# spcl/EBCC

Measured on AMD Instinct MI355X. Metric: fp32 GB/s encode+decode, 721x1440 ERA5 frames MAX_ERROR=0.5, higher is better.
Workload: dtype f32; 1 GPU; 256-frame batch 721x1440 fp32 per GPU, base_cr=30 MAX_ERROR=0.5 (BASELINE configs[1]); frames_per_gpu=256, parallelism=frames sharded over 1 GPU(s), no collective, hw_queues=4, encode_slices=3

## Files before the change

ebcc_amd/csrc/batch_codec.hip:

```cpp
#include "host.hpp"

namespace ebcc {
namespace {

DevRateSearch rate_search_start(float cr0, double q_init, double q_target)
{
    DevRateSearch r{};
    r.lo = r.hi = r.cr = cr0; r.q = r.q0 = q_init; r.qt = q_target;
    r.last.cr = -1; r.last.complete = 1;
    return r;
}

struct Job {
    bool const_field = false;
    float minv = 0, maxv = 0, target = -1, cr = -1;
    double mean_err = 0, q = 0, q_first = 0;
    float rmin = 0, rmax = 0;
    bool skip = true, need_pure = false;
    float best_err = -1;
    size_t coeffs_orig = 0, coeffs_size = 0, len1 = 0;
    double t_hi = 0, t_lo = 0, t_best = 0;
    bool trunc_active = false;
    std::vector<uint8_t> tail, zbytes;
    DevRateSearch rs[2] = {};
    std::vector<DevProbe> probes;
};

struct Batch {
    ebcc_hip_ctx *ctx;
    J2kBuffers &jb;
    const float *d_frames;
    size_t n, tiles, nt;
    std::vector<J2kFrame> jf;
    J2kFrame *tjf;
    std::vector<int> active;
    int *tactive, *ractive;
    std::vector<float> state_cr;
    int *d_active;
    hipStream_t s;
    ebcc_hip_ctx *rc;
    hipStream_t rs;
    Batch(ebcc_hip_ctx *c, const float *d, size_t n_, size_t tiles_ = 1, ebcc_hip_ctx *rc_ = nullptr)
        : ctx(c), jb(*static_cast<J2kBuffers *>(c->j2k)), d_frames(d), n(n_), tiles(tiles_), nt(n_ * tiles_), jf(n_),
          tjf(static_cast<J2kFrame *>(c->h_jf)), active(n_, 0), tactive(c->h_act), ractive(c->h_act + c->max_frames), state_cr(n_, -1.f),
          d_active(c->d_active), s(c->stream), rc(rc_ ? rc_ : c), rs((rc_ ? rc_ : c)->stream)
    {
// ... 26 lines not shown
    {
        for (size_t c = 0; c < n; c++)
            for (size_t t = c * tiles; t < (c + 1) * tiles; t++) tactive[t] = active[c];
        EBCC_HIP_CHECK(hipMemcpyAsync(d_active, tactive, sizeof(int) * nt, hipMemcpyHostToDevice, s));
    }
    void push_ractive()
    {
        for (size_t c = 0; c < n; c++) ractive[c] = active[c];
        EBCC_HIP_CHECK(hipMemcpyAsync(rc->d_active, ractive, sizeof(int) * n, hipMemcpyHostToDevice, rs));
    }
    void allocate()
    {
        push_jf();
        push_active();
        launch_j2k_rate(jb, (int) nt, d_active, s);
    }
    void probe(bool decode)
    {
        allocate();
        if (decode) launch_j2k_probe_decode(d_frames, jb, (int) nt, d_active, s);
        fetch_jf();
    }
    template <class Jobs>
    void collect_tails(Jobs &jobs)
    {
        push_active();
        launch_j2k_write(jb, (int) nt, d_active, s);
        fetch_jf();
        if (tiles == 1) {
            std::vector<size_t> len(n, 0), off(n, 0);
            for (size_t f = 0; f < n; f++) if (active[f]) len[f] = (size_t) jf[f].stream_bytes;
            stage_download(ctx, jb.stream, jb.stream_cap, len.data(), off.data(), n, s);
            for (size_t f = 0; f < n; f++)
                if (active[f]) jobs[f].tail.assign(ctx->h_stage + off[f], ctx->h_stage + off[f] + len[f]);
            return;
        }
        for (size_t c = 0; c < n; c++) {
            if (!active[c]) continue;
            std::vector<uint8_t> &o = jobs[c].tail;
            o.resize((size_t) jf[c].stream_bytes);
            size_t at = kJ2kMainHeaderBytes;
            for (size_t k = 0; k < tiles; k++) {
                const size_t t = c * tiles + k, part = 14 + (size_t) tjf[t].body_bytes;
                const uint8_t *slot = jb.stream + t * jb.stream_cap;
                if (k == 0) EBCC_HIP_CHECK(hipMemcpyAsync(o.data(), slot, kJ2kMainHeaderBytes, hipMemcpyDeviceToHost, s));
                EBCC_HIP_CHECK(hipMemcpyAsync(o.data() + at, slot + kJ2kMainHeaderBytes, part, hipMemcpyDeviceToHost, s));
                at += part;
            }
        }
        wait_stream(s);
        const unsigned H = (unsigned) jb.geom.H;
        for (size_t c = 0; c < n; c++) {
            if (!active[c]) continue;
            std::vector<uint8_t> &o = jobs[c].tail;
            auto put32 = [&](size_t at, unsigned v) { o[at] = (uint8_t) (v >> 24); o[at + 1] = (uint8_t) (v >> 16); o[at + 2] = (uint8_t) (v >> 8); o[at + 3] = (uint8_t) v; };
            put32(12, H * (unsigned) tiles);
            size_t at = kJ2kMainHeaderBytes;
            for (size_t k = 0; k < tiles; k++) {
                o[at + 4] = (uint8_t) (k >> 8); o[at + 5] = (uint8_t) k;
                at += 14 + (size_t) tjf[c * tiles + k].body_bytes;
            }
            o[at] = 0xFF; o[at + 1] = 0xD9;
        }
    }
};

int search_rounds() { const char *e = getenv("EBCC_HIP_SEARCH_ROUNDS"); return e ? std::max(1, atoi(e)) : 16; }
constexpr int kSearchAll = 0, kSearchStart = 1, kSearchFinish = 2;

struct Entropy {
    enum : uint8_t { kNone = 0, kQueued = 1, kRunning = 2, kSkipped = 3 };
    using PoolBatches = std::vector<std::shared_ptr<HostPool::Batch>>;
    std::vector<Job> &jobs;
    const unsigned slices;
    const int level;
    const bool timing, trace;
    std::vector<const uint8_t *> coeff_ptr;
    std::unique_ptr<std::atomic<uint8_t>[]> zstate;
    std::vector<size_t> zfloor;
    std::atomic<long long> zstd_us{0}, zstd_max_us{0}, zstd_bytes{0}, bound_us{0};
    long long wait_us = 0;
    PoolBatches zbatches, fbatches;

    Entropy(std::vector<Job> &j, unsigned slices_, int level_, bool timing_)
        : jobs(j), slices(slices_), level(level_), timing(timing_), trace(timing_ && getenv("EBCC_HIP_ZSTD_TRACE")),
          coeff_ptr(j.size(), nullptr), zstate(new std::atomic<uint8_t>[j.size()]), zfloor(j.size(), 0)
    { for (size_t f = 0; f < j.size(); f++) zstate[f] = kNone; }
    Entropy(const Entropy &) = delete; Entropy &operator=(const Entropy &) = delete;
    ~Entropy() { for (PoolBatches *v : {&fbatches, &zbatches}) for (auto &b : *v) if (b) b->wait(); }

    void submit_zstd(std::vector<size_t> list)
    {
        if (trace) fprintf(stderr, "zstd-submit batch %p jobs %zu\n", (const void *) &jobs, list.size());
        for (size_t f : list) zstate[f] = kQueued;
        auto order = std::make_shared<std::vector<size_t>>(std::move(list));
        zbatches.push_back(HostPool::instance().submit(order->size(), entropy_threads(slices), [this, order](size_t i) {
            const size_t f = (*order)[i];
            uint8_t expect = kQueued;
            if (!zstate[f].compare_exchange_strong(expect, kRunning)) return;
            Job &j = jobs[f];
            const auto z0 = std::chrono::steady_clock::now();
            j.zbytes.resize(zstd().bound(j.coeffs_size));
            const size_t z = zstd().compress(j.zbytes.data(), j.zbytes.size(), coeff_ptr[f], j.coeffs_size, level);
            if ((zstd().is_error && zstd().is_error(z)) || z > j.zbytes.size()) throw std::runtime_error("ZSTD_compress failed on a residual prefix");
            j.zbytes.resize(z);
            const long long us = std::chrono::duration_cast<std::chrono::microseconds>(std::chrono::steady_clock::now() - z0).count();
            if (trace) {
                static const auto epoch = std::chrono::steady_clock::now();
                const long long a = std::chrono::duration_cast<std::chrono::microseconds>(z0 - epoch).count();
                fprintf(stderr, "zstd-job batch %p bytes %zu start %lld us end %lld us cpu %d\n", (const void *) &jobs, j.coeffs_size, a, a + us, sched_getcpu());
            }
            zstd_us += us; zstd_bytes += (long long) j.coeffs_size;
            long long m = zstd_max_us.load(); while (us > m && !zstd_max_us.compare_exchange_weak(m, us)) {}
        }));
    }
    void submit_floors(const std::vector<size_t> &frames)
    {
        auto list = std::make_shared<std::vector<size_t>>(frames);
        fbatches.push_back(HostPool::instance().submit(list->size(), entropy_threads(slices), [this, list](size_t i) {
            const size_t f = (*list)[i];
            const auto z0 = std::chrono::steady_clock::now();
            zfloor[f] = zstd_size_lower_bound(coeff_ptr[f], jobs[f].coeffs_size);
            bound_us += std::chrono::duration_cast<std::chrono::microseconds>(std::chrono::steady_clock::now() - z0).count();
        }));
    }
    std::vector<size_t> longest_first(std::vector<size_t> list) const
    {
        std::stable_sort(list.begin(), list.end(), [&](size_t a, size_t c) { return jobs[a].coeffs_size > jobs[c].coeffs_size; });
        return list;
    }
    std::vector<size_t> lowest_floor_first(std::vector<size_t> list) const
    {
        std::stable_sort(list.begin(), list.end(), [&](size_t a, size_t c) {
            return (double) zfloor[a] * (double) jobs[c].coeffs_size < (double) zfloor[c] * (double) jobs[a].coeffs_size; });
        return list;
    }
// ... 5 lines not shown
    bool floor_decides(size_t f) const { return zfloor[f] > 0 && (size_t) jobs[f].rs[1].last.stream_bytes < zfloor[f] + jobs[f].len1; }
    bool strike(size_t f)
    {
        uint8_t expect = kNone;
        if (zstate[f].compare_exchange_strong(expect, kSkipped)) return true;
        expect = kQueued;
        return zstate[f].compare_exchange_strong(expect, kSkipped);
    }
    bool join(PoolBatches &v)
    {
        const auto w0 = std::chrono::steady_clock::now();
        bool ok = true;
        std::string why;
        for (auto &b : v) if (b && !b->wait()) { ok = false; if (why.empty()) why = b->error; }
        v.clear();
        wait_us += std::chrono::duration_cast<std::chrono::microseconds>(std::chrono::steady_clock::now() - w0).count();
        if (!ok) { log_fatal("entropy stage failed: %s", why.c_str()); set_error("%s", why.c_str()); }
        return ok;
    }
    bool join_floors() { return join(fbatches); }
    bool join_all() { const bool a = join(fbatches), c = join(zbatches); return a && c; }
    void report(const std::vector<size_t> &with_prefix, long long skipped, long long skipped_bytes) const
    {
        if (timing) fprintf(stderr, "ebcc-mi355x zstd: %.1f ms of core time for %lld bytes, longest job %.1f ms; floors %.1f ms; %lld of %zu prefixes (%lld bytes) not compressed\n",
                            zstd_us.load() / 1e3, zstd_bytes.load(), zstd_max_us.load() / 1e3, bound_us.load() / 1e3, skipped, with_prefix.size(), skipped_bytes);
        host_stats().skipped_bytes += skipped_bytes;
        if (trace)
            for (size_t f : with_prefix) {
                const Job &j = jobs[f];
                const long long x = (long long) j.rs[1].last.stream_bytes - (long long) j.len1;
                fprintf(stderr, "zstd-trace c %zu floor %zu X %lld z %zu state %d need_pure %d nbad1 %llu len1 %zu orig %zu\n", j.coeffs_size, zfloor[f], x, j.zbytes.size(), (int) zstate[f].load(), (int) j.need_pure,
                        (unsigned long long) j.rs[0].last.nbad, j.len1, j.coeffs_orig);
            }
    }
};

struct BatchEncode {
    struct Gate { SliceGate *g; void release() { if (g) { g->release(); g = nullptr; } } ~Gate() { release(); } } next;
    struct NoteOnce { PhaseNote *n; void tell() { if (n) { n->slice_done(); n = nullptr; } } ~NoteOnce() { tell(); } } gpu_phase_over;
    const EncodeEnv env;
    const codec_config_t *cfg;
    const int mode;
    const bool searching;
    const double q_target;
    const bool want_pure;
    const size_t n, n_pix;
    const unsigned slices;
    Batch b;
    const bool overlap2;
    std::vector<Job> jobs;
    PhaseTimer pt;
    bool any_resid = false;
    bool search2_queued = false;

    BatchEncode(ebcc_hip_ctx *ctx, const float *d_frames, size_t n_, const codec_config_t *cfg_, SliceGate *next_, size_t tiles,
                ebcc_hip_ctx *rctx, unsigned slices_, PhaseNote *note)
        : next{next_}, gpu_phase_over{note}, cfg(cfg_), mode((int) cfg_->residual_compression_type),
          searching(mode == MAX_ERROR || mode == RELATIVE_ERROR), q_target(1 - env.base_error_quantile),
          want_pure(q_target != 1.0 && !env.no_fallback), n(n_), n_pix(ctx->n_pix * tiles), slices(slices_),
          b(ctx, d_frames, n_, tiles, rctx), overlap2(want_pure && tiles == 1 && b.rc == ctx), jobs(n_) {}
    ~BatchEncode() { if (search2_queued && b.ctx->stream2) hipStreamSynchronize(b.ctx->stream2); }

    int analyse(); void first_probe(); void search_1(); void queue_search_2(); bool residual_layer(); void truncation_search();
    bool entropy_and_fallback(); int assemble(uint8_t **outs, size_t *sizes);
    void start_search_2();
    void rate_search(int k, int lane = 0, int part = kSearchAll);
};

void BatchEncode::rate_search(int k, int lane, int part)
{
    ebcc_hip_ctx *ctx = b.ctx;
    DevChunk *h = static_cast<DevChunk *>(ctx->h_search) + (size_t) lane * ctx->max_frames, *d = static_cast<DevChunk *>(ctx->d_search) + (size_t) lane * ctx->max_frames;
    int *const d_counter = ctx->d_counter + 4 * lane, *const h_counter = ctx->h_counter + 4 * lane;
    int *const d_active = lane ? ctx->d_active + ctx->max_frames : b.d_active;
    hipStream_t s = lane ? second_stream(ctx) : b.s;
    J2kBuffers &jb = b.jb;
    const int forced = getenv("EBCC_HIP_SPECULATION") ? atoi(getenv("EBCC_HIP_SPECULATION")) != 0 : -1;
    const bool speculate = lane == 0 && (forced >= 0 ? forced != 0 : slices <= 1);
    hipStream_t s2 = nullptr;
    double jobs_qt0 = 0.0;
    for (size_t f = 0; f < n; f++) if (!jobs[f].const_field) { jobs_qt0 = jobs[f].rs[0].qt; break; }
    const double limit_qt = getenv("EBCC_HIP_NO_SHORTCUTS") || g_log_level <= 0 ? 0.0 : std::min(jobs_qt0, 1.0);
    auto advance = [&]() {
        launch_search_advance(d, jb.jf, d_active, (int) n, (int) b.tiles, k, (double) n_pix, d_counter, s,
                              speculate ? jb.cand_cr : nullptr, speculate ? jb.cand_sel : nullptr, limit_qt);
        if (speculate) launch_j2k_rate_publish(jb, (int) b.nt, s);
    };
// ... 274 lines not shown
            drive(forced_rounds ? search_rounds() : cuts_left + 1, 6, [&] {
                launch_prefix_synthesis_stats(b.d_frames, b.jb.DEC, rc->rb, (int) n, rc->d_u64b, rc->d_active, rs);
                advance();
            });
        }
        for (size_t f = 0; f < n; f++) {
            Job &j = jobs[f];
            const DevChunk &c = h[f];
            if (j.trunc_active) { j.t_hi = c.t_hi; j.t_lo = c.t_lo; j.t_best = c.t_best; j.mean_err = c.mean_err; j.best_err = c.best_err; }
            j.trunc_active = false;
        }
    }
    for (Job &j : jobs) {
        if (j.const_field || j.skip) j.coeffs_size = j.need_pure ? j.coeffs_orig : 0;
        else j.coeffs_size = (size_t) (j.t_best / 8.);
    }
    pt.mark("truncation search");
}

bool BatchEncode::entropy_and_fallback()
{
    ebcc_hip_ctx *rc = b.rc;
    Entropy es(jobs, slices, env.zstd_level, pt.on);
    std::vector<size_t> coeff_len(n, 0), coeff_off(n, 0);
    for (size_t f = 0; f < n; f++) {
        if (jobs[f].coeffs_size <= 16) jobs[f].coeffs_size = 0;
        coeff_len[f] = jobs[f].coeffs_size;
    }
    stage_download(rc, (const uint8_t *) rc->rb.stream, rc->rb.stream_words * sizeof(uint32_t), coeff_len.data(), coeff_off.data(), n, b.rs);
    std::vector<size_t> with_prefix;
    for (size_t f = 0; f < n; f++)
        if (coeff_len[f]) { es.coeff_ptr[f] = rc->h_stage + coeff_off[f]; with_prefix.push_back(f); }
    std::vector<size_t> cand;
    if (!want_pure) {
        es.submit_zstd(es.longest_first(with_prefix));
    } else {
        const bool use_floor = zstd_floor_usable() && !getenv("EBCC_HIP_NO_SHORTCUTS");
        std::vector<size_t> now;
        for (size_t f : with_prefix) {
            if (jobs[f].need_pure) { es.zstate[f] = Entropy::kSkipped; continue; }
            (use_floor && jobs[f].coeffs_size <= kZstdFloorMaxBytes ? cand : now).push_back(f);
        }
        if (!now.empty()) es.submit_zstd(es.longest_first(now));
        if (!cand.empty()) es.submit_floors(cand);
    }
    pt.mark("zstd: queued");
    if (want_pure) {
        if (overlap2) {
            rate_search(1, 1, kSearchFinish);
            search2_queued = false;
            pt.mark("rate search 2");
            gpu_phase_over.tell();
            if (!es.join_floors()) return false;
        } else {
            start_search_2();
            rate_search(1, 0, kSearchStart);
            if (!cand.empty()) {
                if (!es.join_floors()) return false;
                es.submit_zstd(es.lowest_floor_first(cand));
            }
            rate_search(1, 0, kSearchFinish);
            pt.mark("rate search 2");
            gpu_phase_over.tell();
        }
        long long skipped_bytes = 0, skipped = 0;
        for (size_t f : cand)
            if (es.floor_decides(f) && es.strike(f)) { skipped++; skipped_bytes += (long long) jobs[f].coeffs_size; }
        if (overlap2) {
            const std::vector<size_t> open = es.not_started(cand);
            if (!open.empty()) es.submit_zstd(es.longest_first(open));
        }
        if (!es.join_all()) return false;
        pt.mark("zstd: wait for the workers");
        for (size_t f : with_prefix) if (jobs[f].need_pure) { skipped++; skipped_bytes += (long long) jobs[f].coeffs_size; }
        es.report(with_prefix, skipped, skipped_bytes);
        bool any_pure = false;
        for (size_t f = 0; f < n; f++) {
            Job &j = jobs[f];
            b.active[f] = 0;
            if (j.const_field) continue;
            const size_t len2 = (size_t) j.rs[1].last.stream_bytes;
            const bool decided = es.floor_decides(f);
            if (decided || len2 < j.zbytes.size() + j.len1 || j.need_pure) {
                if (decided) log_info("frame %zu: pure base compression (%zu) beats base (%zu) + residual (at least %zu)", f, len2, j.len1, es.zfloor[f]);
                else if (len2 < j.zbytes.size() + j.len1)
                    log_info("frame %zu: pure base compression (%zu) beats base (%zu) + residual (%zu)", f, len2, j.len1, j.zbytes.size());
                j.mean_err = j.rs[1].last.err_sum / (double) n_pix;
                j.zbytes.clear(); j.coeffs_size = 0;
                b.active[f] = 1; b.jf[f].cr = j.rs[1].result; any_pure = true;
            }
        }
        if (any_pure) { b.allocate(); b.collect_tails(jobs); }
    }
    if (!es.join_all()) return false;
    host_stats().add(es.zstd_us.load() + es.bound_us.load(), es.wait_us, es.zstd_bytes.load());
    return true;
}

int BatchEncode::assemble(uint8_t **outs, size_t *sizes)
{
    for (size_t f = 0; f < n; f++) {
        Job &j = jobs[f];
        float minv = j.minv, maxv = j.maxv;
        log_info("frame %zu: mean of compression error %e", f, j.mean_err);
        if (!env.no_mean_adjust && std::fabs(j.mean_err) > 1e-18) {
            minv += j.mean_err;
            maxv += j.mean_err;
        }
        const size_t codec_size = j.const_field ? sizeof(uint64_t) : j.tail.size();
        const size_t total = sizeof(FrameHeader) + j.zbytes.size() + codec_size;
        uint8_t *o = (uint8_t *) malloc(total), *p = o;
        if (!o) { log_fatal("out of memory"); return 1; }
        FrameHeader hd;
        memset(&hd, 0, sizeof hd);
        memcpy(hd.magic, EBCC_HEADER_MAGIC, 4);
        hd.version = EBCC_HEADER_VERSION;
        if (j.const_field) hd.flags |= EBCC_HEADER_FLAG_CONST_FIELD;
        hd.minval_bits = f2u(minv); hd.maxval_bits = f2u(maxv);
        hd.coeffs_size = j.coeffs_size;
        hd.rmin_bits = f2u(j.const_field ? 0.0f : j.rmin); hd.rmax_bits = f2u(j.const_field ? 0.0f : j.rmax);
        hd.compressed_size = j.zbytes.size(); hd.tail_size = codec_size;
        memcpy(p, &hd, sizeof hd); p += sizeof hd;
        if (!j.zbytes.empty()) { memcpy(p, j.zbytes.data(), j.zbytes.size()); p += j.zbytes.size(); }
        if (j.const_field) { uint64_t cnt = n_pix; memcpy(p, &cnt, 8); }
        else memcpy(p, j.tail.data(), j.tail.size());
        log_info("frame %zu: coeffs_size %zu compressed_size %zu jp2_length %zu ratio %f", f, j.coeffs_size, j.zbytes.size(),
                 codec_size, (double) (n_pix * 4) / (double) total);
        outs[f] = o;
        sizes[f] = total;
    }
    pt.mark("assemble");
    return 0;
}

}

int encode_batch(ebcc_hip_ctx *ctx, const float *d_frames, size_t n, const codec_config_t *cfg, uint8_t **outs, size_t *sizes,
                 SliceGate *next, size_t tiles, ebcc_hip_ctx *rctx, unsigned slices, PhaseNote *note)
{
    BatchEncode e(ctx, d_frames, n, cfg, next, tiles, rctx, slices, note);
    if (const int r = e.analyse()) return r;
    e.first_probe();
    if (e.searching) {
        e.search_1();
        e.queue_search_2();
        if (!e.residual_layer()) return 1;
        e.truncation_search();
        if (!e.entropy_and_fallback()) return 1;
    }
    e.pt.mark("fallback search + tails");
    return e.assemble(outs, sizes);
}
// ... 240 lines not shown
```

ebcc_amd/csrc/engine.hip:

```cpp
#include "engine.hpp"

#include <algorithm>
#include <atomic>
#include <cstdarg>
#include <mutex>
#include <string>
#include <type_traits>
#include <cstring>
#include <vector>

#include "../../include/ebcc_hip.h"
#include "search.hpp"

namespace ebcc {

static thread_local std::string g_last_error;

void set_error(const char *fmt, ...)
{
    char buf[512];
    va_list ap;
    va_start(ap, fmt);
    vsnprintf(buf, sizeof buf, fmt, ap);
    va_end(ap);
// ... 58 lines not shown
template float *ctx_alloc<float>(ebcc_hip_ctx *, size_t);
template int32_t *ctx_alloc<int32_t>(ebcc_hip_ctx *, size_t);
template uint32_t *ctx_alloc<uint32_t>(ebcc_hip_ctx *, size_t);
template uint16_t *ctx_alloc<uint16_t>(ebcc_hip_ctx *, size_t);
template uint8_t *ctx_alloc<uint8_t>(ebcc_hip_ctx *, size_t);
template double *ctx_alloc<double>(ebcc_hip_ctx *, size_t);
template unsigned long long *ctx_alloc<unsigned long long>(ebcc_hip_ctx *, size_t);
template FrameState *ctx_alloc<FrameState>(ebcc_hip_ctx *, size_t);

namespace {

__global__ __launch_bounds__(256) void k_stage(uint8_t *slots, size_t stride, const unsigned long long *pack, uint8_t *staged, int to_stage)
{
    const int f = blockIdx.x;
    const unsigned long long off = pack[2 * f], len = pack[2 * f + 1];
    if (!len) return;
    uint32_t *a = (uint32_t *) (slots + (size_t) f * stride), *b = (uint32_t *) (staged + off);
    const size_t words = (size_t) ((len + 3) / 4);
    for (size_t i = (size_t) blockIdx.y * blockDim.x + threadIdx.x; i < words; i += (size_t) gridDim.y * blockDim.x) {
        if (to_stage) b[i] = a[i]; else a[i] = b[i];
    }
}

size_t stage_layout(ebcc_hip_ctx *ctx, const size_t *len, size_t *off, size_t n)
{
    size_t total = 0;
    for (size_t f = 0; f < n; f++) {
        off[f] = total;
        ctx->h_pack[2 * f] = total; ctx->h_pack[2 * f + 1] = len[f];
        total += (len[f] + 15) & ~(size_t) 15;
    }
    if (total > ctx->stage_cap) {
        uint8_t *h_old = ctx->h_stage, *d_old = ctx->d_stage;
        ctx->h_stage = nullptr; ctx->d_stage = nullptr; ctx->stage_cap = 0;
        if (h_old) hipHostFree(h_old);
        if (d_old) hipFree(d_old);
        const size_t cap = total + total / 2 + 4096;
        uint8_t *h_new = nullptr, *d_new = nullptr;
        EBCC_HIP_CHECK(hipHostMalloc((void **) &h_new, cap));
        const hipError_t e = device_malloc((void **) &d_new, cap);
        if (e != hipSuccess) { hipHostFree(h_new); EBCC_HIP_CHECK(e); }
        ctx->h_stage = h_new; ctx->d_stage = d_new; ctx->stage_cap = cap;
        poison_alloc(d_new, cap);
    }
    return total;
}

}

void stage_download(ebcc_hip_ctx *ctx, const uint8_t *src, size_t stride, const size_t *len, size_t *off, size_t n, hipStream_t s)
{
    const size_t total = stage_layout(ctx, len, off, n);
    if (!total) return;
    EBCC_HIP_CHECK(hipMemcpyAsync(ctx->d_pack, ctx->h_pack, 2 * n * sizeof(unsigned long long), hipMemcpyHostToDevice, s));
    hipLaunchKernelGGL(k_stage, dim3((unsigned) n, 4), dim3(256), 0, s, const_cast<uint8_t *>(src), stride, ctx->d_pack, ctx->d_stage, 1);
    EBCC_HIP_CHECK(hipMemcpyAsync(ctx->h_stage, ctx->d_stage, total, hipMemcpyDeviceToHost, s));
    wait_stream(s);
}

void stage_reserve(ebcc_hip_ctx *ctx, const size_t *len, size_t *off, size_t m) { stage_layout(ctx, len, off, m); }

void stage_send(ebcc_hip_ctx *ctx, size_t m, hipStream_t s)
{
    size_t total = 0;
    for (size_t k = 0; k < m; k++) total = std::max<size_t>(total, ctx->h_pack[2 * k] + ((ctx->h_pack[2 * k + 1] + 15) & ~15ull));
    EBCC_HIP_CHECK(hipMemcpyAsync(ctx->d_pack, ctx->h_pack, 2 * m * sizeof(unsigned long long), hipMemcpyHostToDevice, s));
    if (total) EBCC_HIP_CHECK(hipMemcpyAsync(ctx->d_stage, ctx->h_stage, total, hipMemcpyHostToDevice, s));
}

void stage_scatter(ebcc_hip_ctx *ctx, uint8_t *dst, size_t stride, size_t first, size_t count, hipStream_t s)
{
    if (!count) return;
    hipLaunchKernelGGL(k_stage, dim3((unsigned) count, 4), dim3(256), 0, s, dst, stride, ctx->d_pack + 2 * first, ctx->d_stage, 0);
}

bool ensure_cut_slots(ebcc_hip_ctx *ctx, int capacity)
{
    if (ctx->cut.capacity >= capacity) return true;
    if (ctx->cut_failed) return false;
    const int cap = capacity;
// ... 201 lines not shown
{
    EBCC_API_TRY
    if (!ctx) return;
    hipSetDevice(ctx->device);
    if (ctx->stream) hipStreamSynchronize(ctx->stream);
    for (ebcc_hip_ctx *c : ctx->lanes) ebcc_hip_destroy(c);
    ctx->lanes.clear();
    if (ctx->twin) { ebcc_hip_destroy(ctx->twin); ctx->twin = nullptr; }
    j2k_destroy(ctx);
    for (void *p : ctx->allocs) hipFree(p);
    if (ctx->h_u64a) hipHostFree(ctx->h_u64a);
    if (ctx->h_u64b) hipHostFree(ctx->h_u64b);
    if (ctx->h_u64c) hipHostFree(ctx->h_u64c);
    if (ctx->h_active) hipHostFree(ctx->h_active);
    if (ctx->h_fs) hipHostFree(ctx->h_fs);
    if (ctx->h_pack) hipHostFree(ctx->h_pack);
    if (ctx->h_act) hipHostFree(ctx->h_act);
    if (ctx->h_search) hipHostFree(ctx->h_search);
    if (ctx->h_counter) hipHostFree(ctx->h_counter);
    if (ctx->h_jf) hipHostFree(ctx->h_jf);
    if (ctx->h_table) hipHostFree(ctx->h_table);
    if (ctx->h_stage) hipHostFree(ctx->h_stage);
    if (ctx->d_stage) hipFree(ctx->d_stage);
    if (ctx->d_io) hipFree(ctx->d_io);
    if (ctx->h_boxes) hipHostFree(ctx->h_boxes);
    if (ctx->d_boxes) hipFree(ctx->d_boxes);
    if (ctx->h_bounce) hipHostFree(ctx->h_bounce);
    if (ctx->ev_a) hipEventDestroy(ctx->ev_a);
    if (ctx->ev_b) hipEventDestroy(ctx->ev_b);
    if (ctx->stream2) hipStreamDestroy(ctx->stream2);
    if (ctx->stream) hipStreamDestroy(ctx->stream);
    delete ctx;
    EBCC_API_CATCH_VOID
}

void *ebcc_hip_stream(ebcc_hip_ctx *ctx) { return ctx ? (void *) ctx->stream : nullptr; }
size_t ebcc_hip_workspace_bytes(const ebcc_hip_ctx *ctx) { return ctx ? ctx->bytes : 0; }
size_t ebcc_hip_padded_pixels(const ebcc_hip_ctx *ctx) { return ctx ? ctx->rb.np : 0; }

void *ebcc_hip_malloc(size_t bytes)
{
    void *p = nullptr;
    if (device_malloc(&p, bytes ? bytes : 1) != hipSuccess) {
        set_error("ebcc_hip_malloc(%zu) failed", bytes);
        return nullptr;
    }
// ... 149 lines not shown
```

ebcc_amd/csrc/engine.hpp:

```cpp
#pragma once

#include <cstdint>
#include <string>
#include <vector>

#include "residual.hpp"

struct ebcc_hip_ctx {
    int device = 0;
    hipStream_t stream = nullptr;
    size_t max_frames = 0;
    int height = 0, width = 0;
    int tile_period = 1;
    size_t n_pix = 0;
    size_t bytes = 0;
    ebcc::ResidualBuffers rb{};
    unsigned long long *d_u64a = nullptr, *d_u64b = nullptr, *d_u64c = nullptr;
    int *d_active = nullptr;
    unsigned long long *h_u64a = nullptr, *h_u64b = nullptr, *h_u64c = nullptr;
    int *h_active = nullptr;
    ebcc::FrameState *h_fs = nullptr;
    void *h_jf = nullptr;
    int *h_act = nullptr;
    int *h_table = nullptr;
    void *d_search = nullptr, *h_search = nullptr;
    int *d_counter = nullptr, *h_counter = nullptr;
    std::vector<void *> allocs;
    void *j2k = nullptr;
    hipStream_t stream2 = nullptr;
    hipEvent_t ev_a = nullptr, ev_b = nullptr;
    std::vector<ebcc_hip_ctx *> lanes;
    ebcc_hip_ctx *twin = nullptr;
    bool twin_failed = false;
    uint8_t *h_stage = nullptr, *d_stage = nullptr;
    size_t stage_cap = 0;
    float *d_io = nullptr;
    size_t io_cap = 0;
    uint8_t *h_bounce = nullptr;
    unsigned long long *h_pack = nullptr, *d_pack = nullptr;
    void *h_boxes = nullptr, *d_boxes = nullptr;
    size_t boxes_cap = 0;
    ebcc::CutSlots cut{};
    bool cut_failed = false;
};

namespace ebcc {

void set_error(const char *fmt, ...);
ebcc_hip_ctx *create_engine(int device, size_t max_frames, size_t height, size_t width, int tile_period);
template <typename T>
T *ctx_alloc(ebcc_hip_ctx *ctx, size_t count);

void stage_download(ebcc_hip_ctx *ctx, const uint8_t *src, size_t stride, const size_t *len, size_t *off, size_t n, hipStream_t s);
void stage_reserve(ebcc_hip_ctx *ctx, const size_t *len, size_t *off, size_t m);
void stage_send(ebcc_hip_ctx *ctx, size_t m, hipStream_t s);
void stage_scatter(ebcc_hip_ctx *ctx, uint8_t *dst, size_t stride, size_t first, size_t count, hipStream_t s);

bool ensure_cut_slots(ebcc_hip_ctx *ctx, int capacity);

int check_ims_header(ebcc_hip_ctx *ctx, const uint8_t *b, size_t n, size_t num_bits);

void fetch_frame_states(ebcc_hip_ctx *ctx, size_t n_frames);
void push_frame_states(ebcc_hip_ctx *ctx, size_t n_frames, hipStream_t s = nullptr);

}
```

ebcc_amd/csrc/host.hpp:

```cpp
#pragma once

#include <dlfcn.h>

#include <chrono>
#include <cmath>
#include <cstdarg>
#include <cstring>
#include <ctime>
#include <sched.h>
#include <condition_variable>
#include <deque>
#include <functional>
#include <map>
#include <sys/mman.h>
#include <sys/resource.h>
#include <sys/syscall.h>
#include <unistd.h>
#include <tuple>
#include <algorithm>
#include <atomic>
#include <mutex>
#include <memory>
#include <thread>
#include <string>
#include <vector>

#include "../../include/ebcc_hip.h"
#include "engine.hpp"
#include "j2k.hpp"
#include "search.hpp"


namespace ebcc {

bool j2k_parse_codestream(const uint8_t *cs, size_t n, const J2kGeom &g, int *table);
bool j2k_peek_dims(const uint8_t *cs, size_t n, int *W, int *H, int *tile_w, int *tile_h);
bool j2k_parse_tiled(const uint8_t *cs, size_t n, const J2kBuffers &jb, int tiles, int *tables, size_t *part_off, size_t *part_len);

extern int g_log_level;
void log_at(int level, const char *fmt, ...);
#define log_trace(...) ::ebcc::log_at(0, __VA_ARGS__)
#define log_info(...) ::ebcc::log_at(2, __VA_ARGS__)
#define log_warn(...) ::ebcc::log_at(3, __VA_ARGS__)
#define log_fatal(...) ::ebcc::log_at(5, __VA_ARGS__)

struct Zstd {
    size_t (*bound)(size_t) = nullptr;
    size_t (*compress)(void *, size_t, const void *, size_t, int) = nullptr;
    size_t (*decompress)(void *, size_t, const void *, size_t) = nullptr;
    unsigned (*is_error)(size_t) = nullptr;
    unsigned (*version)(void) = nullptr;
    bool ok = false;
    Zstd();
};
Zstd &zstd();
constexpr size_t kZstdFloorMaxBytes = (size_t) 4 << 20;
bool zstd_floor_usable();
size_t zstd_size_lower_bound(const uint8_t *src, size_t n);

#pragma pack(push, 1)
struct FrameHeader {
    uint8_t magic[4]; uint8_t version; uint8_t flags; uint16_t reserved;
    uint32_t minval_bits, maxval_bits; uint64_t coeffs_size;
    uint32_t rmin_bits, rmax_bits; uint64_t compressed_size; uint64_t tail_size;
};
struct ChunkHeader {
    uint8_t magic[4]; uint32_t version, ndims, reserved;
    uint64_t dims[3], chunk_dims[3], num_chunks, chunk_size;
};
#pragma pack(pop)
static_assert(sizeof(FrameHeader) == 48, "EBCC header must be 48 bytes");
static_assert(sizeof(ChunkHeader) == 80, "EBCK header must be 80 bytes");
inline uint32_t f2u(float f) { uint32_t u; memcpy(&u, &f, 4); return u; }
inline float u2f(uint32_t u) { float f; memcpy(&f, &u, 4); return f; }

inline bool dims_are_valid(const size_t d[3])
{
    if (d[0] == 0 || d[1] == 0) return false;
    size_t hh = d[0] * d[1];
    if (hh / d[0] != d[1]) return false;
    return hh >= EBCC_MIN_INTERNAL_IMAGE_DIM && hh <= EBCC_MAX_INTERNAL_IMAGE_DIM && d[2] >= EBCC_MIN_INTERNAL_IMAGE_DIM &&
           d[2] <= EBCC_MAX_INTERNAL_IMAGE_DIM;
}

struct EncodeEnv {
    double base_error_quantile = 1e-6;
    bool no_fallback = false, no_consistency = false, no_mean_adjust = false;
    int zstd_level = 22;
    EncodeEnv()
    {
        if (const char *e = getenv("EBCC_INIT_BASE_ERROR_QUANTILE")) base_error_quantile = strtod(e, nullptr);
        no_fallback = getenv("EBCC_DISABLE_PURE_BASE_COMPRESSION_FALLBACK") != nullptr;
        no_consistency = getenv("EBCC_DISABLE_PURE_BASE_COMPRESSION_FALLBACK_CONSISTENCY") != nullptr;
        no_mean_adjust = getenv("EBCC_DISABLE_MEAN_ADJUSTMENT") != nullptr;
        if (const char *e = getenv("EBCC_ZSTD_LEVEL")) { long v = strtol(e, nullptr, 10); if (v >= 1 && v <= 22) zstd_level = (int) v; }
    }
};
// ... 13 lines not shown
struct SliceGate {
    std::mutex m;
    std::condition_variable cv;
    bool open = false;
    void release() { { std::lock_guard<std::mutex> l(m); open = true; } cv.notify_all(); }
    void wait() { std::unique_lock<std::mutex> l(m); cv.wait(l, [&] { return open; }); }
};

constexpr int kJ2kMainHeaderBytes = 135;

inline hipStream_t second_stream(ebcc_hip_ctx *c)
{
    if (!c->stream2) EBCC_HIP_CHECK(hipStreamCreateWithFlags(&c->stream2, hipStreamNonBlocking));
    return c->stream2;
}

double cgroup_cpu_quota();
unsigned usable_cpus();
unsigned entropy_threads_for(unsigned cpus, unsigned local_world, unsigned slices);
unsigned entropy_threads(unsigned slices = 1);

struct HostStats {
    std::atomic<long long> zstd_core_us{0}, zstd_wait_us{0}, zstd_bytes{0}, batches{0}, skipped_bytes{0};
    void add(long long core_us, long long wait_us, long long bytes) { zstd_core_us += core_us; zstd_wait_us += wait_us; zstd_bytes += bytes; batches++; }
    void reset() { zstd_core_us = 0; zstd_wait_us = 0; zstd_bytes = 0; batches = 0; skipped_bytes = 0; }
};
HostStats &host_stats();

class HostPool {
  public:
    struct Batch {
        std::function<void(size_t)> fn;
        size_t n = 0;
        std::atomic<size_t> next{0};
        std::atomic<size_t> left{0};
        std::atomic<bool> failed{false};
        std::string error;
        std::mutex m;
        std::condition_variable cv;
        void fail(const char *what) { std::lock_guard<std::mutex> l(m); if (!failed.exchange(true)) error = what; }
        bool wait()
        {
            work();
            std::unique_lock<std::mutex> l(m);
            cv.wait(l, [&] { return left.load() == 0; });
            return !failed.load();
        }
        void work()
// ... 105 lines not shown
```

ebcc_amd/csrc/host_codec.hip:

```cpp
#include "host.hpp"

using namespace ebcc;

namespace {

int resolve_device()
{
    int n = 0;
    if (hipGetDeviceCount(&n) != hipSuccess || n < 1) return 0;
    if (const char *e = getenv("EBCC_HIP_DEVICE")) { int d = atoi(e); return d >= 0 && d < n ? d : 0; }
    int d = 0;
    if (hipGetDevice(&d) != hipSuccess) d = 0;
    return d;
}
bool multi_process_job()
{
    for (const char *v : {"LOCAL_WORLD_SIZE", "WORLD_SIZE"})
        if (const char *e = getenv(v)) if (atoi(e) > 1) return true;
    return false;
}
std::vector<int> device_list()
{
    int n = 0;
    if (hipGetDeviceCount(&n) != hipSuccess || n < 1) return {0};
// ... 593 lines not shown
{
    static const char *names[] = {"NONE", "MAX_ERROR", "RELATIVE_ERROR"};
    log_info("dimensions:\t(%lu, %lu, %lu)", c->dims[0], c->dims[1], c->dims[2]);
    log_info("chunk dimensions:\t(%lu, %lu, %lu)", c->chunk_dims[0], c->chunk_dims[1], c->chunk_dims[2]);
    log_info("base_cr:\t%f", c->base_cr);
    unsigned t = (unsigned) c->residual_compression_type;
    log_info("residual type:\t%s", t < 3 ? names[t] : "?");
    if (t == MAX_ERROR) log_info("max error:\t%f", c->error);
    if (t == RELATIVE_ERROR) log_info("relative error:\t%f", c->error);
}

int ebcc_hip_host_threads(int slices) { return (int) entropy_threads((unsigned) std::max(1, slices)); }
int ebcc_hip_default_encode_slices(void) { return (int) default_encode_slices(); }
int ebcc_hip_encode_slices_for(size_t n_frames) { return (int) slice_count(n_frames, "EBCC_HIP_SLICES", default_encode_slices()); }

int ebcc_hip_selfcheck(void) { return j2k_selfcheck_div65535() + residual_selfcheck_divisions(); }
void ebcc_hip_plan_decode_lanes(const int *table, int n_code_blocks, int out[4]) { plan_decode_lanes(table, std::max(0, n_code_blocks), out); }

size_t ebcc_hip_zstd_floor(const uint8_t *src, size_t n) { return zstd_floor_usable() ? zstd_size_lower_bound(src, n) : 0; }

void ebcc_hip_host_stats(double *out, int reset)
{
    HostStats &h = host_stats();
    if (out) {
        out[0] = (double) usable_cpus(); out[1] = cgroup_cpu_quota();
        out[2] = h.zstd_core_us.load() / 1e6; out[3] = h.zstd_wait_us.load() / 1e6;
        out[4] = (double) h.zstd_bytes.load(); out[5] = (double) h.batches.load(); out[6] = (double) h.skipped_bytes.load();
    }
    if (reset) h.reset();
}

int ebcc_hip_upload(ebcc_hip_ctx *ctx, void *d_dst, const void *h_src, size_t bytes)
{
    if (!ctx || !d_dst || !h_src) { set_error("ebcc_hip_upload: null argument"); return 1; }
    return on_device(ctx->device, 1, [&] {
        copy_pageable(ctx, const_cast<void *>(h_src), d_dst, bytes, false);
        return 0;
    });
}
int ebcc_hip_download(ebcc_hip_ctx *ctx, void *h_dst, const void *d_src, size_t bytes)
{
    if (!ctx || !h_dst || !d_src) { set_error("ebcc_hip_download: null argument"); return 1; }
    return on_device(ctx->device, 1, [&] {
        huge_pages(h_dst, bytes);
        copy_pageable(ctx, h_dst, const_cast<void *>(d_src), bytes, true);
        return 0;
// ... 376 lines not shown
```

Baseline: 8.807 GB/s.

## Download pure codestreams early and assemble frames while zstd workers run

While zstd workers are still compressing residuals, the encoder now downloads the pure-base codestreams into a second staging buffer. It then assembles each frame as soon as both its payload and pure stream are ready, using a per-frame latch, so the choice and header assembly overlap with entropy coding instead of running after the join. This avoids a later GPU pass for fallback frames and moves assembly off the critical path. The cost is a speculative download of pure streams that may go unused, an extra pinned staging buffer, and assembly running from worker threads.

```diff
diff --git a/ebcc_amd/csrc/batch_codec.hip b/ebcc_amd/csrc/batch_codec.hip
--- a/ebcc_amd/csrc/batch_codec.hip
+++ b/ebcc_amd/csrc/batch_codec.hip
@@ -22,6 +22,12 @@
     double t_hi = 0, t_lo = 0, t_best = 0;
     bool trunc_active = false;
     std::vector<uint8_t> tail, zbytes;
+    const uint8_t *tail_pure = nullptr;
+    size_t tail_pure_len = 0;
+    FrameLatch latch;
+    uint8_t *out = nullptr;
+    size_t out_size = 0;
+    bool out_pure = false;
     DevRateSearch rs[2] = {};
     std::vector<DevProbe> probes;
 };
@@ -94,7 +100,7 @@
         fetch_jf();
     }
     template <class Jobs>
-    void collect_tails(Jobs &jobs)
+    size_t collect_tails(Jobs &jobs, bool beside = false)
     {
         push_active();
         launch_j2k_write(jb, (int) nt, d_active, s);
@@ -102,10 +108,16 @@
         if (tiles == 1) {
             std::vector<size_t> len(n, 0), off(n, 0);
             for (size_t f = 0; f < n; f++) if (active[f]) len[f] = (size_t) jf[f].stream_bytes;
+            if (beside) {
+                const size_t total = stage_download(ctx, jb.stream, jb.stream_cap, len.data(), off.data(), n, s, true);
+                for (size_t f = 0; f < n; f++)
+                    if (active[f]) { jobs[f].tail_pure = ctx->h_stage2 + off[f]; jobs[f].tail_pure_len = len[f]; }
+                return total;
+            }
             stage_download(ctx, jb.stream, jb.stream_cap, len.data(), off.data(), n, s);
             for (size_t f = 0; f < n; f++)
                 if (active[f]) jobs[f].tail.assign(ctx->h_stage + off[f], ctx->h_stage + off[f] + len[f]);
-            return;
+            return 0;
         }
         for (size_t c = 0; c < n; c++) {
             if (!active[c]) continue;
@@ -134,6 +146,7 @@
             }
             o[at] = 0xFF; o[at + 1] = 0xD9;
         }
+        return 0;
     }
 };
 
@@ -150,8 +163,9 @@
     std::vector<const uint8_t *> coeff_ptr;
     std::unique_ptr<std::atomic<uint8_t>[]> zstate;
     std::vector<size_t> zfloor;
-    std::atomic<long long> zstd_us{0}, zstd_max_us{0}, zstd_bytes{0}, bound_us{0};
+    std::atomic<long long> zstd_us{0}, zstd_max_us{0}, zstd_bytes{0}, bound_us{0}, zstd_jobs{0};
     long long wait_us = 0;
+    std::function<void(size_t)> payload_ready;
     PoolBatches zbatches, fbatches;
 
     Entropy(std::vector<Job> &j, unsigned slices_, int level_, bool timing_)
@@ -182,8 +196,9 @@
                 const long long a = std::chrono::duration_cast<std::chrono::microseconds>(z0 - epoch).count();
                 fprintf(stderr, "zstd-job batch %p bytes %zu start %lld us end %lld us cpu %d\n", (const void *) &jobs, j.coeffs_size, a, a + us, sched_getcpu());
             }
-            zstd_us += us; zstd_bytes += (long long) j.coeffs_size;
+            zstd_us += us; zstd_bytes += (long long) j.coeffs_size; zstd_jobs++;
             long long m = zstd_max_us.load(); while (us > m && !zstd_max_us.compare_exchange_weak(m, us)) {}
+            if (payload_ready) payload_ready(f);
         }));
     }
     void submit_floors(const std::vector<size_t> &frames)
@@ -235,8 +250,8 @@
     bool join_all() { const bool a = join(fbatches), c = join(zbatches); return a && c; }
     void report(const std::vector<size_t> &with_prefix, long long skipped, long long skipped_bytes) const
     {
-        if (timing) fprintf(stderr, "ebcc-mi355x zstd: %.1f ms of core time for %lld bytes, longest job %.1f ms; floors %.1f ms; %lld of %zu prefixes (%lld bytes) not compressed\n",
-                            zstd_us.load() / 1e3, zstd_bytes.load(), zstd_max_us.load() / 1e3, bound_us.load() / 1e3, skipped, with_prefix.size(), skipped_bytes);
+        if (timing) fprintf(stderr, "ebcc-mi355x zstd: %.1f ms of core time for %lld bytes in %lld jobs, longest job %.1f ms; floors %.1f ms; %lld of %zu prefixes (%lld bytes) not compressed\n",
+                            zstd_us.load() / 1e3, zstd_bytes.load(), zstd_jobs.load(), zstd_max_us.load() / 1e3, bound_us.load() / 1e3, skipped, with_prefix.size(), skipped_bytes);
         host_stats().skipped_bytes += skipped_bytes;
         if (trace)
             for (size_t f : with_prefix) {
@@ -272,10 +287,17 @@
           searching(mode == MAX_ERROR || mode == RELATIVE_ERROR), q_target(1 - env.base_error_quantile),
           want_pure(q_target != 1.0 && !env.no_fallback), n(n_), n_pix(ctx->n_pix * tiles), slices(slices_),
           b(ctx, d_frames, n_, tiles, rctx), overlap2(want_pure && tiles == 1 && b.rc == ctx), jobs(n_) {}
-    ~BatchEncode() { if (search2_queued && b.ctx->stream2) hipStreamSynchronize(b.ctx->stream2); }
+    ~BatchEncode()
+    {
+        if (search2_queued && b.ctx->stream2) hipStreamSynchronize(b.ctx->stream2);
+        for (Job &j : jobs) free(j.out);
+    }
 
     int analyse(); void first_probe(); void search_1(); void queue_search_2(); bool residual_layer(); void truncation_search();
     bool entropy_and_fallback(); int assemble(uint8_t **outs, size_t *sizes);
+    FrameParts parts_of(const Job &j, bool pure) const;
+    void assemble_one(size_t f, bool pure);
+    void assemble_chosen(size_t f);
     void start_search_2();
     void rate_search(int k, int lane = 0, int part = kSearchAll);
 };
@@ -596,6 +618,9 @@
 {
     ebcc_hip_ctx *rc = b.rc;
     Entropy es(jobs, slices, env.zstd_level, pt.on);
+    const bool early = overlap2 && !getenv("EBCC_HIP_NO_SHORTCUTS");
+    size_t early_bytes = 0;
+    if (early) es.payload_ready = [this](size_t f) { if (jobs[f].latch.arrive(FrameLatch::kPayload)) assemble_chosen(f); };
     std::vector<size_t> coeff_len(n, 0), coeff_off(n, 0);
     for (size_t f = 0; f < n; f++) {
         if (jobs[f].coeffs_size <= 16) jobs[f].coeffs_size = 0;
@@ -624,7 +649,7 @@
             rate_search(1, 1, kSearchFinish);
             search2_queued = false;
             pt.mark("rate search 2");
-            gpu_phase_over.tell();
+            if (!early) gpu_phase_over.tell();
             if (!es.join_floors()) return false;
         } else {
             start_search_2();
@@ -644,15 +669,49 @@
             const std::vector<size_t> open = es.not_started(cand);
             if (!open.empty()) es.submit_zstd(es.longest_first(open));
         }
+        if (early) {
+            std::vector<float> cr_before(n, 0.f);
+            std::vector<uint8_t> has_job(n, 0), pure_now(n, 0);
+            bool any = false;
+            for (size_t f = 0; f < n; f++) {
+                const Job &j = jobs[f];
+                b.active[f] = 0;
+                if (j.const_field) continue;
+                const uint8_t st = es.zstate[f].load();
+                has_job[f] = st == Entropy::kQueued || st == Entropy::kRunning;
+                pure_now[f] = !has_job[f] && (j.need_pure || es.floor_decides(f) || pure_base_wins((size_t) j.rs[1].last.stream_bytes, 0, j.len1));
+                if (has_job[f] || pure_now[f]) { b.active[f] = 1; cr_before[f] = b.jf[f].cr; b.jf[f].cr = j.rs[1].result; any = true; }
+            }
+            if (any) { b.allocate(); early_bytes = b.collect_tails(jobs, true); }
+            for (size_t f = 0; f < n; f++)
+                if (b.active[f]) { b.jf[f].cr = cr_before[f]; b.active[f] = 0; }
+            gpu_phase_over.tell();
+            pt.mark("pure codestreams, early");
+            for (size_t f = 0; f < n; f++)
+                if (has_job[f] && jobs[f].latch.arrive(FrameLatch::kPure)) assemble_chosen(f);
+            for (size_t f = 0; f < n; f++)
+                if (!has_job[f]) assemble_one(f, pure_now[f] != 0);
+            pt.mark("assembly in the wait");
+        }
         if (!es.join_all()) return false;
         pt.mark("zstd: wait for the workers");
         for (size_t f : with_prefix) if (jobs[f].need_pure) { skipped++; skipped_bytes += (long long) jobs[f].coeffs_size; }
         es.report(with_prefix, skipped, skipped_bytes);
+        if (early && pt.on) fprintf(stderr, "ebcc-mi355x early pure codestreams: %zu bytes downloaded\n", early_bytes);
         bool any_pure = false;
         for (size_t f = 0; f < n; f++) {
             Job &j = jobs[f];
             b.active[f] = 0;
             if (j.const_field) continue;
+            if (j.out) {
+                if (j.out_pure) {
+                    const size_t len2 = (size_t) j.rs[1].last.stream_bytes;
+                    if (es.floor_decides(f)) log_info("frame %zu: pure base compression (%zu) beats base (%zu) + residual (at least %zu)", f, len2, j.len1, es.zfloor[f]);
+                    else if (!j.need_pure) log_info("frame %zu: pure base compression (%zu) beats base (%zu) + residual (%zu)", f, len2, j.len1, j.zbytes.size());
+                    j.mean_err = j.rs[1].last.err_sum / (double) n_pix; j.zbytes.clear(); j.coeffs_size = 0;
+                }
+                continue;
+            }
             const size_t len2 = (size_t) j.rs[1].last.stream_bytes;
             const bool decided = es.floor_decides(f);
             if (decided || len2 < j.zbytes.size() + j.len1 || j.need_pure) {
@@ -667,41 +726,59 @@
         if (any_pure) { b.allocate(); b.collect_tails(jobs); }
     }
     if (!es.join_all()) return false;
-    host_stats().add(es.zstd_us.load() + es.bound_us.load(), es.wait_us, es.zstd_bytes.load());
+    host_stats().add(es.zstd_us.load() + es.bound_us.load(), es.wait_us, es.zstd_bytes.load(), es.zstd_jobs.load(), es.zstd_max_us.load());
     return true;
+}
+
+FrameParts BatchEncode::parts_of(const Job &j, bool pure) const
+{
+    FrameParts fp;
+    fp.const_field = j.const_field; fp.no_mean_adjust = env.no_mean_adjust;
+    fp.minv = j.minv; fp.maxv = j.maxv; fp.rmin = j.rmin; fp.rmax = j.rmax;
+    fp.n_pix = n_pix;
+    if (pure) {
+        fp.mean_err = j.rs[1].last.err_sum / (double) n_pix;
+        fp.tail = j.tail_pure; fp.tail_len = j.tail_pure_len;
+    } else {
+        fp.mean_err = j.mean_err;
+        fp.coeffs_size = j.coeffs_size;
+        fp.z = j.zbytes.data(); fp.z_len = j.zbytes.size();
+        fp.tail = j.tail.data(); fp.tail_len = j.tail.size();
+    }
+    return fp;
+}
+
+void BatchEncode::assemble_one(size_t f, bool pure)
+{
+    Job &j = jobs[f];
+    j.out = assemble_frame(parts_of(j, pure), &j.out_size);
+    j.out_pure = pure;
+    if (!j.out) throw std::runtime_error("out of memory");
+}
+
+void BatchEncode::assemble_chosen(size_t f)
+{
+    Job &j = jobs[f];
+    j.out = assemble_choice(parts_of(j, false), parts_of(j, true), j.len1, (size_t) j.rs[1].last.stream_bytes, &j.out_pure, &j.out_size);
+    if (!j.out) throw std::runtime_error("out of memory");
 }
 
 int BatchEncode::assemble(uint8_t **outs, size_t *sizes)
 {
     for (size_t f = 0; f < n; f++) {
         Job &j = jobs[f];
-        float minv = j.minv, maxv = j.maxv;
         log_info("frame %zu: mean of compression error %e", f, j.mean_err);
-        if (!env.no_mean_adjust && std::fabs(j.mean_err) > 1e-18) {
-            minv += j.mean_err;
-            maxv += j.mean_err;
-        }
-        const size_t codec_size = j.const_field ? sizeof(uint64_t) : j.tail.size();
-        const size_t total = sizeof(FrameHeader) + j.zbytes.size() + codec_size;
-        uint8_t *o = (uint8_t *) malloc(total), *p = o;
-        if (!o) { log_fatal("out of memory"); return 1; }
-        FrameHeader hd;
-        memset(&hd, 0, sizeof hd);
-        memcpy(hd.magic, EBCC_HEADER_MAGIC, 4);
-        hd.version = EBCC_HEADER_VERSION;
-        if (j.const_field) hd.flags |= EBCC_HEADER_FLAG_CONST_FIELD;
-        hd.minval_bits = f2u(minv); hd.maxval_bits = f2u(maxv);
-        hd.coeffs_size = j.coeffs_size;
-        hd.rmin_bits = f2u(j.const_field ? 0.0f : j.rmin); hd.rmax_bits = f2u(j.const_field ? 0.0f : j.rmax);
-        hd.compressed_size = j.zbytes.size(); hd.tail_size = codec_size;
-        memcpy(p, &hd, sizeof hd); p += sizeof hd;
-        if (!j.zbytes.empty()) { memcpy(p, j.zbytes.data(), j.zbytes.size()); p += j.zbytes.size(); }
-        if (j.const_field) { uint64_t cnt = n_pix; memcpy(p, &cnt, 8); }
-        else memcpy(p, j.tail.data(), j.tail.size());
+        if (!j.out) {
+            j.out = assemble_frame(parts_of(j, false), &j.out_size);
+            if (!j.out) { log_fatal("out of memory"); return 1; }
+        }
+        const size_t codec_size = j.out_size - sizeof(FrameHeader) - j.zbytes.size();
         log_info("frame %zu: coeffs_size %zu compressed_size %zu jp2_length %zu ratio %f", f, j.coeffs_size, j.zbytes.size(),
-                 codec_size, (double) (n_pix * 4) / (double) total);
-        outs[f] = o;
-        sizes[f] = total;
+                 codec_size, (double) (n_pix * 4) / (double) j.out_size);
+    }
+    for (size_t f = 0; f < n; f++) {
+        outs[f] = jobs[f].out; sizes[f] = jobs[f].out_size;
+        jobs[f].out = nullptr;
     }
     pt.mark("assemble");
     return 0;
diff --git a/ebcc_amd/csrc/engine.hip b/ebcc_amd/csrc/engine.hip
--- a/ebcc_amd/csrc/engine.hip
+++ b/ebcc_amd/csrc/engine.hip
@@ -104,17 +104,19 @@
     }
 }
 
-size_t stage_layout(ebcc_hip_ctx *ctx, const size_t *len, size_t *off, size_t n)
-{
+size_t stage_layout(ebcc_hip_ctx *ctx, const size_t *len, size_t *off, size_t n, bool second = false)
+{
+    uint8_t *&h_stage = second ? ctx->h_stage2 : ctx->h_stage, *&d_stage = second ? ctx->d_stage2 : ctx->d_stage;
+    size_t &stage_cap = second ? ctx->stage2_cap : ctx->stage_cap;
     size_t total = 0;
     for (size_t f = 0; f < n; f++) {
         off[f] = total;
         ctx->h_pack[2 * f] = total; ctx->h_pack[2 * f + 1] = len[f];
         total += (len[f] + 15) & ~(size_t) 15;
     }
-    if (total > ctx->stage_cap) {
-        uint8_t *h_old = ctx->h_stage, *d_old = ctx->d_stage;
-        ctx->h_stage = nullptr; ctx->d_stage = nullptr; ctx->stage_cap = 0;
+    if (total > stage_cap) {
+        uint8_t *h_old = h_stage, *d_old = d_stage;
+        h_stage = nullptr; d_stage = nullptr; stage_cap = 0;
         if (h_old) hipHostFree(h_old);
         if (d_old) hipFree(d_old);
         const size_t cap = total + total / 2 + 4096;
@@ -122,7 +124,7 @@
         EBCC_HIP_CHECK(hipHostMalloc((void **) &h_new, cap));
         const hipError_t e = device_malloc((void **) &d_new, cap);
         if (e != hipSuccess) { hipHostFree(h_new); EBCC_HIP_CHECK(e); }
-        ctx->h_stage = h_new; ctx->d_stage = d_new; ctx->stage_cap = cap;
+        h_stage = h_new; d_stage = d_new; stage_cap = cap;
         poison_alloc(d_new, cap);
     }
     return total;
@@ -130,14 +132,16 @@
 
 }
 
-void stage_download(ebcc_hip_ctx *ctx, const uint8_t *src, size_t stride, const size_t *len, size_t *off, size_t n, hipStream_t s)
-{
-    const size_t total = stage_layout(ctx, len, off, n);
-    if (!total) return;
+size_t stage_download(ebcc_hip_ctx *ctx, const uint8_t *src, size_t stride, const size_t *len, size_t *off, size_t n, hipStream_t s, bool second)
+{
+    const size_t total = stage_layout(ctx, len, off, n, second);
+    if (!total) return 0;
+    uint8_t *const h_stage = second ? ctx->h_stage2 : ctx->h_stage, *const d_stage = second ? ctx->d_stage2 : ctx->d_stage;
     EBCC_HIP_CHECK(hipMemcpyAsync(ctx->d_pack, ctx->h_pack, 2 * n * sizeof(unsigned long long), hipMemcpyHostToDevice, s));
-    hipLaunchKernelGGL(k_stage, dim3((unsigned) n, 4), dim3(256), 0, s, const_cast<uint8_t *>(src), stride, ctx->d_pack, ctx->d_stage, 1);
-    EBCC_HIP_CHECK(hipMemcpyAsync(ctx->h_stage, ctx->d_stage, total, hipMemcpyDeviceToHost, s));
+    hipLaunchKernelGGL(k_stage, dim3((unsigned) n, 4), dim3(256), 0, s, const_cast<uint8_t *>(src), stride, ctx->d_pack, d_stage, 1);
+    EBCC_HIP_CHECK(hipMemcpyAsync(h_stage, d_stage, total, hipMemcpyDeviceToHost, s));
     wait_stream(s);
+    return total;
 }
 
 void stage_reserve(ebcc_hip_ctx *ctx, const size_t *len, size_t *off, size_t m) { stage_layout(ctx, len, off, m); }
@@ -385,6 +389,8 @@
     if (ctx->h_table) hipHostFree(ctx->h_table);
     if (ctx->h_stage) hipHostFree(ctx->h_stage);
     if (ctx->d_stage) hipFree(ctx->d_stage);
+    if (ctx->h_stage2) hipHostFree(ctx->h_stage2);
+    if (ctx->d_stage2) hipFree(ctx->d_stage2);
     if (ctx->d_io) hipFree(ctx->d_io);
     if (ctx->h_boxes) hipHostFree(ctx->h_boxes);
     if (ctx->d_boxes) hipFree(ctx->d_boxes);
diff --git a/ebcc_amd/csrc/engine.hpp b/ebcc_amd/csrc/engine.hpp
--- a/ebcc_amd/csrc/engine.hpp
+++ b/ebcc_amd/csrc/engine.hpp
@@ -34,6 +34,8 @@
     bool twin_failed = false;
     uint8_t *h_stage = nullptr, *d_stage = nullptr;
     size_t stage_cap = 0;
+    uint8_t *h_stage2 = nullptr, *d_stage2 = nullptr;
+    size_t stage2_cap = 0;
     float *d_io = nullptr;
     size_t io_cap = 0;
     uint8_t *h_bounce = nullptr;
@@ -51,7 +53,7 @@
 template <typename T>
 T *ctx_alloc(ebcc_hip_ctx *ctx, size_t count);
 
-void stage_download(ebcc_hip_ctx *ctx, const uint8_t *src, size_t stride, const size_t *len, size_t *off, size_t n, hipStream_t s);
+size_t stage_download(ebcc_hip_ctx *ctx, const uint8_t *src, size_t stride, const size_t *len, size_t *off, size_t n, hipStream_t s, bool second = false);
 void stage_reserve(ebcc_hip_ctx *ctx, const size_t *len, size_t *off, size_t m);
 void stage_send(ebcc_hip_ctx *ctx, size_t m, hipStream_t s);
 void stage_scatter(ebcc_hip_ctx *ctx, uint8_t *dst, size_t stride, size_t first, size_t count, hipStream_t s);
diff --git a/ebcc_amd/csrc/frame_assembly.hpp b/ebcc_amd/csrc/frame_assembly.hpp
--- /dev/null
+++ b/ebcc_amd/csrc/frame_assembly.hpp
@@ -0,0 +1,81 @@
+#pragma once
+
+#include <atomic>
+#include <cmath>
+#include <cstdint>
+#include <cstdlib>
+#include <cstring>
+
+#include "../../include/ebcc_codec.h"
+
+namespace ebcc {
+
+#pragma pack(push, 1)
+struct FrameHeader {
+    uint8_t magic[4]; uint8_t version; uint8_t flags; uint16_t reserved;
+    uint32_t minval_bits, maxval_bits; uint64_t coeffs_size;
+    uint32_t rmin_bits, rmax_bits; uint64_t compressed_size; uint64_t tail_size;
+};
+#pragma pack(pop)
+static_assert(sizeof(FrameHeader) == 48, "EBCC header must be 48 bytes");
+inline uint32_t f2u(float f) { uint32_t u; memcpy(&u, &f, 4); return u; }
+inline float u2f(uint32_t u) { float f; memcpy(&f, &u, 4); return f; }
+
+struct FrameParts {
+    bool const_field = false, no_mean_adjust = false;
+    float minv = 0, maxv = 0, rmin = 0, rmax = 0;
+    double mean_err = 0;
+    size_t coeffs_size = 0;
+    const uint8_t *z = nullptr; size_t z_len = 0;
+    const uint8_t *tail = nullptr; size_t tail_len = 0;
+    uint64_t n_pix = 0;
+};
+
+inline bool pure_base_wins(size_t len2, size_t z, size_t len1) { return len2 < z + len1; }
+
+inline uint8_t *assemble_frame(const FrameParts &fp, size_t *total_out)
+{
+    float minv = fp.minv, maxv = fp.maxv;
+    if (!fp.no_mean_adjust && std::fabs(fp.mean_err) > 1e-18) {
+        minv += fp.mean_err;
+        maxv += fp.mean_err;
+    }
+    const size_t codec_size = fp.const_field ? sizeof(uint64_t) : fp.tail_len;
+    const size_t total = sizeof(FrameHeader) + fp.z_len + codec_size;
+    uint8_t *o = (uint8_t *) malloc(total), *p = o;
+    if (!o) return nullptr;
+    FrameHeader hd;
+    memset(&hd, 0, sizeof hd);
+    memcpy(hd.magic, EBCC_HEADER_MAGIC, 4);
+    hd.version = EBCC_HEADER_VERSION;
+    if (fp.const_field) hd.flags |= EBCC_HEADER_FLAG_CONST_FIELD;
+    hd.minval_bits = f2u(minv); hd.maxval_bits = f2u(maxv);
+    hd.coeffs_size = fp.coeffs_size;
+    hd.rmin_bits = f2u(fp.const_field ? 0.0f : fp.rmin); hd.rmax_bits = f2u(fp.const_field ? 0.0f : fp.rmax);
+    hd.compressed_size = fp.z_len; hd.tail_size = codec_size;
+    memcpy(p, &hd, sizeof hd); p += sizeof hd;
+    if (fp.z_len) { memcpy(p, fp.z, fp.z_len); p += fp.z_len; }
+    if (fp.const_field) { uint64_t cnt = fp.n_pix; memcpy(p, &cnt, 8); }
+    else if (fp.tail_len) memcpy(p, fp.tail, fp.tail_len);
+    *total_out = total;
+    return o;
+}
+
+struct FrameLatch {
+    enum : unsigned { kPayload = 1, kPure = 2 };
+    std::atomic<unsigned> got{0};
+    bool arrive(unsigned input)
+    {
+        const unsigned before = got.fetch_or(input, std::memory_order_acq_rel);
+        return !(before & input) && (before | input) == (kPayload | kPure);
+    }
+    bool complete() const { return got.load(std::memory_order_acquire) == (kPayload | kPure); }
+};
+
+inline uint8_t *assemble_choice(const FrameParts &residual, const FrameParts &pure, size_t len1, size_t len2, bool *took_pure, size_t *total_out)
+{
+    *took_pure = pure_base_wins(len2, residual.z_len, len1);
+    return assemble_frame(*took_pure ? pure : residual, total_out);
+}
+
+}
diff --git a/ebcc_amd/csrc/host.hpp b/ebcc_amd/csrc/host.hpp
--- a/ebcc_amd/csrc/host.hpp
+++ b/ebcc_amd/csrc/host.hpp
@@ -27,6 +27,7 @@
 
 #include "../../include/ebcc_hip.h"
 #include "engine.hpp"
+#include "frame_assembly.hpp"
 #include "j2k.hpp"
 #include "search.hpp"
 
@@ -59,20 +60,12 @@
 size_t zstd_size_lower_bound(const uint8_t *src, size_t n);
 
 #pragma pack(push, 1)
-struct FrameHeader {
-    uint8_t magic[4]; uint8_t version; uint8_t flags; uint16_t reserved;
-    uint32_t minval_bits, maxval_bits; uint64_t coeffs_size;
-    uint32_t rmin_bits, rmax_bits; uint64_t compressed_size; uint64_t tail_size;
-};
 struct ChunkHeader {
     uint8_t magic[4]; uint32_t version, ndims, reserved;
     uint64_t dims[3], chunk_dims[3], num_chunks, chunk_size;
 };
 #pragma pack(pop)
-static_assert(sizeof(FrameHeader) == 48, "EBCC header must be 48 bytes");
 static_assert(sizeof(ChunkHeader) == 80, "EBCK header must be 80 bytes");
-inline uint32_t f2u(float f) { uint32_t u; memcpy(&u, &f, 4); return u; }
-inline float u2f(uint32_t u) { float f; memcpy(&f, &u, 4); return f; }
 
 inline bool dims_are_valid(const size_t d[3])
 {
@@ -132,8 +125,13 @@
 
 struct HostStats {
     std::atomic<long long> zstd_core_us{0}, zstd_wait_us{0}, zstd_bytes{0}, batches{0}, skipped_bytes{0};
-    void add(long long core_us, long long wait_us, long long bytes) { zstd_core_us += core_us; zstd_wait_us += wait_us; zstd_bytes += bytes; batches++; }
-    void reset() { zstd_core_us = 0; zstd_wait_us = 0; zstd_bytes = 0; batches = 0; skipped_bytes = 0; }
+    std::atomic<long long> zstd_jobs{0}, zstd_longest_us{0};
+    void add(long long core_us, long long wait_us, long long bytes, long long jobs = 0, long long longest_us = 0)
+    {
+        zstd_core_us += core_us; zstd_wait_us += wait_us; zstd_bytes += bytes; batches++; zstd_jobs += jobs;
+        long long m = zstd_longest_us.load(); while (longest_us > m && !zstd_longest_us.compare_exchange_weak(m, longest_us)) {}
+    }
+    void reset() { zstd_core_us = 0; zstd_wait_us = 0; zstd_bytes = 0; batches = 0; skipped_bytes = 0; zstd_jobs = 0; zstd_longest_us = 0; }
 };
 HostStats &host_stats();
 
diff --git a/ebcc_amd/csrc/host_codec.hip b/ebcc_amd/csrc/host_codec.hip
--- a/ebcc_amd/csrc/host_codec.hip
+++ b/ebcc_amd/csrc/host_codec.hip
@@ -639,6 +639,9 @@
 void ebcc_hip_host_stats(double *out, int reset)
 {
     HostStats &h = host_stats();
+    if (getenv("EBCC_HIP_PHASE_TIMING"))
+        fprintf(stderr, "ebcc-mi355x host stats: %lld zstd jobs in %lld entropy batches, longest job %.1f ms, %.1f ms of core time, %.1f ms of waiting\n",
+                h.zstd_jobs.load(), h.batches.load(), h.zstd_longest_us.load() / 1e3, h.zstd_core_us.load() / 1e3, h.zstd_wait_us.load() / 1e3);
     if (out) {
         out[0] = (double) usable_cpus(); out[1] = cgroup_cpu_quota();
         out[2] = h.zstd_core_us.load() / 1e6; out[3] = h.zstd_wait_us.load() / 1e6;
```

Result: no change. 8.892 GB/s (median of 6 runs) (+1.0%).
